# SingleZombie/AFLDM

Measured on AMD Instinct MI355X. Metric: denoise-steps/sec + ms/step, FFHQ-256 AF-UNet, batch 64 @1/2/4/8 GPU, higher is better.
Workload: dtype bf16; 1 GPU; FFHQ-256 AF-UNet single denoise step, batch 64 per GPU (BASELINE configs[1]); batch_per_gpu=64, global_batch=64, hip_graph=True, latents_finite=True

## Files before the change

afldm_amd/_lib.py:

```python
import ctypes
import os
from ctypes import POINTER, Structure, c_char_p, c_float, c_int, c_longlong, c_size_t, c_void_p

import torch

F32, BF16 = 0, 1
DTYPE_CODE = {torch.float32: F32, torch.bfloat16: BF16}

_HERE = os.path.dirname(os.path.abspath(__file__))
LIB_PATH = os.environ.get("AFLDM_LIB") or os.path.join(_HERE, "lib", "libafldm_hip.so")


class ConvArgs(Structure):
    _fields_ = [
        ("x1", c_void_p), ("x2", c_void_p), ("w", c_void_p), ("bias", c_void_p), ("temb", c_void_p),
        ("residual", c_void_p), ("y", c_void_p), ("workspace", c_void_p), ("workspace_bytes", c_size_t),
        ("C1", c_int), ("C2", c_int), ("B", c_int), ("H", c_int), ("W", c_int), ("Cout", c_int),
        ("KS", c_int), ("temb_stride", c_int), ("res_ld", c_int), ("y_ld", c_int),
        ("out_mode", c_int), ("dtype", c_int), ("y2", c_void_p), ("split_n", c_int),
        ("stats_out", c_void_p), ("temb_mod", c_int), ("sync", c_void_p), ("sync_bytes", c_size_t),
        ("defer_reduce", c_int), ("w_batch_stride", ctypes.c_longlong),
        ("y_norm", c_void_p), ("norm_gamma", c_void_p), ("norm_beta", c_void_p), ("norm_groups", c_int), ("norm_eps", c_float),
        ("x_layout", c_int), ("y_layout", c_int),
    ]


class AfActArgs(Structure):
    _fields_ = [
        ("x1", c_void_p), ("x2", c_void_p), ("C1", c_int), ("C2", c_int), ("stats1", c_void_p), ("S1", c_int),
        ("stats2", c_void_p), ("S2", c_int), ("gamma", c_void_p), ("beta", c_void_p), ("G", c_int), ("eps", c_float),
        ("U", c_void_p), ("D", c_void_p), ("packed", c_void_p),
    ]


class SepArgs(Structure):
    _fields_ = [
        ("x", c_void_p), ("y", c_void_p), ("M", c_void_p), ("M2", c_void_p), ("gn_table", c_void_p),
        ("outer_count", ctypes.c_longlong), ("inner_count", ctypes.c_longlong),
# ... 42 lines not shown
        "afldm_af_resample_plane": ([vp, vp, vp, vp, ip, ip, ip, ip, ip, vp], c_int),
        "afldm_upfirdn2d": ([vp, vp, vp] + [ip] * 14 + [fp, ip, vp], c_int),
        "afldm_upfirdn2d_out_size": ([ip] * 6, c_int),
        "afldm_masked_metrics": ([vp, vp, vp, vp, ip, c_size_t, ip, vp], c_int),
        "afldm_gn_fold": ([vp, ip, vp, ip, ip, ip, vp], c_int),
        "afldm_gn_table": ([vp, ip, vp, vp, vp, ip, ip, ip, ip, fp, vp], c_int),
        "afldm_softmax_rows": ([vp, vp, ctypes.c_longlong, ip, fp, ip, vp], c_int),
        "afldm_conv2d": ([POINTER(ConvArgs), vp], c_int),
        "afldm_conv2d_workspace": ([POINTER(ConvArgs)], c_size_t),
        "afldm_conv2d_stats_splits": ([POINTER(ConvArgs)], c_int),
        "afldm_conv2d_tune": ([ip, ip], c_int),
        "afldm_conv2d_fused_splitk": ([ip], c_int),
        "afldm_conv2d_variant": ([POINTER(ConvArgs)], c_int),
        "afldm_conv2d_c8_ok": ([POINTER(ConvArgs)], c_int),
        "afldm_conv2d_norm_ok": ([POINTER(ConvArgs)], c_int),
        "afldm_conv2d_s2": ([POINTER(ConvArgs), ip, ip, vp], c_int),
        "afldm_conv2d_up2": ([POINTER(ConvArgs), vp], c_int),
        "afldm_conv2d_s2_stats_splits": ([POINTER(ConvArgs)], c_int),
        "afldm_conv2d_up2_stats_splits": ([POINTER(ConvArgs)], c_int),
        "afldm_pack_weight_up2": ([vp, vp, ip, ip, ip, vp], c_int),
        "afldm_attention": ([vp, ip, vp, ip, vp, vp, ip, ip, ip, ip, ip, ip, ip, fp, ip, vp], c_int),
        "afldm_attn_block_fused_supported": ([ip, ip, ip, ip], c_int),
        "afldm_attn_block_fused_trace": ([vp], c_int),
        "afldm_af_act_trace": ([vp], c_int),
        "afldm_attn_block_fused": ([vp, vp, ip, vp, vp, ip, fp, vp, vp, vp, ip, ip, ip, ip, fp, ip, vp], c_int),
        "afldm_attn_block_fused_out_supported": ([ip, ip, ip, ip, ip], c_int),
        "afldm_attn_block_fused_out": ([vp, vp, ip, vp, vp, ip, fp, vp, vp, vp, vp, vp, vp, vp, vp, c_longlong, ip, ip, ip, ip, fp, ip,
                                        vp], c_int),
        "afldm_ddim_step": ([vp, vp, vp, vp, vp, ip, ip, ip, ip, ip, ip, vp], c_int),
        "afldm_ddim_step_flat": ([vp, vp, vp, fp, fp, fp, fp, c_size_t, vp], c_int),
# ... 45 lines not shown
```

afldm_amd/csrc/conv.hip:

```cpp
#include <stdlib.h>

#include "conv_common.hpp"

namespace afldm {

__device__ __forceinline__ int swz(int row) { return (4 - ((row >> 2) & 3)) & 3; }

template <typename T>
__device__ __forceinline__ void epilogue_store(const ConvP& p, int m, int n, f32x4 v) {
  const T* temb = (const T*)p.temb;
  const T* res = (const T*)p.residual;
  T* y = (T*)p.y;
  const int HW = p.H * p.W;
  const int b = m / HW;
  if (p.y2 && n >= p.split_n) {
    T* y2 = (T*)p.y2;
    const int pix = m - b * HW, c2 = p.Cout - p.split_n;
    for (int r = 0; r < 4 && n + r < p.Cout; ++r) {
      float sv = v[r] + (p.bias ? p.bias[n + r] : 0.f);
      y2[((size_t)b * c2 + (n + r - p.split_n)) * HW + pix] = from_f32<T>(sv);
    }
    return;
  }
  if (n + 3 < p.Cout && p.vec_ok) {
// ... 1848 lines not shown
    p.stage_ok = ((a->out_mode == 1 || a->y_ld % eo == 0) && (!a->residual || a->res_ld % eo == 0) &&
                  (!a->temb || a->temb_stride % eo == 0) && (!cm || hw % eo == 0) && (!a->y2 || a->split_n % eo == 0) &&
                  !(cm && a->residual)) ? 1 : 0;
    static const int s_nostage = getenv("AFLDM_CONV_NOSTAGE") ? atoi(getenv("AFLDM_CONV_NOSTAGE")) : 0;
    if (s_nostage) p.stage_ok = 0;
  }
  {
    static const int s_mfast = getenv("AFLDM_CONV_MFAST") ? atoi(getenv("AFLDM_CONV_MFAST")) : -1;
    p.m_fast = s_mfast >= 0 ? s_mfast : ((long long)a->Cout * a->KS * a->KS > (long long)p.M ? 1 : 0);
  }
  p.xcd_gn = 0;
  p.y_norm = nullptr; p.ngamma = nullptr; p.nbeta = nullptr; p.ncpg = 1; p.neps = 0.f;
  p.x_c8 = a->x_layout == 1 ? 1 : 0;
  p.y_c8 = a->y_layout == 1 ? 1 : 0;
  p.w_nt = 0;
}

template <typename T>
static bool c8_ok(const afldm_conv_args* a) {
  if (sizeof(T) != 2 || a->C2 != 0 || a->x2 || a->y2 || a->out_mode != 0 || a->y_norm || a->y_ld != a->Cout || a->Cout % 8 || a->C1 % 64) return false;
  if (a->w_batch_stride || a->defer_reduce || a->KS != 3 || lin_wreg_bm(a) || skinny_stats_splits(a)) return false;
  const Exec ex = resolve_exec<T>(a);
  if (ex.pl.kind != 0 || kVariants[ex.vid].ver != 6 || ex.splitk != 1 || ex.fused) return false;
  if (a->stats_out) {
    int S = 0;
    if (stats_mode<T>(a, ex, &S) != ST_EPILOGUE) return false;
  }
  return a->H == a->W && a->W <= 32 && a->H * a->W >= kVariants[ex.vid].bm;
}

template <typename T>
static int conv_dispatch(const afldm_conv_args* a, hipStream_t st) {
  AFLDM_REQUIRE((a->x_layout == 0 && a->y_layout == 0) || c8_ok<T>(a), AFLDM_ESHAPE,
                "afldm_conv2d: x_layout / y_layout = 1 (8-channel blocks) is not available for this problem (afldm_conv2d_c8_ok)");
  ConvP p;
  fill_convp<T>(a, p);
  const Exec ex = resolve_exec<T>(a);
  const Plan& pl = ex.pl;
  int smode = 0;
  p.stats_out = nullptr;
  p.stats_S = 1;
  p.stats_multi = 0;
  if (a->stats_out) smode = stats_mode<T>(a, ex, &p.stats_S);
  int rc = AFLDM_OK;
  AFLDM_REQUIRE(!a->w_batch_stride || pl.kind == 0, AFLDM_ESHAPE, "afldm_conv2d: w_batch_stride needs the GEMM path (Cin a multiple of the K step)");
  if (lin_wreg_bm(a)) return lin_wreg_launch(a, st);
  if (skinny_stats_splits(a)) return skinny_launch(a, st);
  if (pl.kind == 1 && cin4_mfma_ok<T>(a)) {
    if (smode == ST_EPILOGUE) p.stats_out = a->stats_out;
// ... 127 lines not shown
  const long long per = (long long)a->H * a->W * (a->C1 > a->C2 ? a->C1 : a->C2) * esz;
  if (a->B <= 1 || (long long)a->B * per < (1ll << 31) || per >= (1ll << 31)) return a->B;
  int c = (int)(((1ll << 31) - 1) / per);
  while (c > 1 && a->B % c) --c;
  return c;
}

static afldm_conv_args conv_chunk_args(const afldm_conv_args* a, int c) {
  afldm_conv_args q = *a;
  q.B = c;
  return q;
}

template <typename T>
static bool plan_h3(const afldm_conv_args* a, ConvP& p, int& vid) {
  if (conv_batch_chunk(a) != a->B || a->w_batch_stride || a->defer_reduce || a->KS != 3) return false;
  if (lin_wreg_bm(a) || skinny_stats_splits(a)) return false;
  fill_convp<T>(a, p);
  const Exec ex = resolve_exec<T>(a);
  if (ex.pl.kind != 0 || kVariants[ex.vid].ver != 6 || ex.splitk != 1 || ex.fused) return false;
  p.stats_out = nullptr;
  p.stats_S = 1;
  p.stats_multi = 0;
  if (a->stats_out) {
    if (stats_mode<T>(a, ex, &p.stats_S) != ST_EPILOGUE) return false;
    p.stats_out = a->stats_out;
    p.stats_multi = (a->H * a->W) == 1 ? 2 : (a->H * a->W) < kVariants[ex.vid].bm ? 1 : 0;
  }
  p.ksteps = 9 * ((a->C1 + a->C2) / (KCH_DEFAULT * epr<T>()));
  p.splitk = 1;
  p.sync = nullptr;
// ... 21 lines not shown

extern "C" int afldm_conv2d_c8_ok(const afldm_conv_args* a) {
  if (!a || a->dtype != AFLDM_BF16 || conv_validate(a) || conv_batch_chunk(a) != a->B) return 0;
  return c8_ok<bf16>(a) ? 1 : 0;
}

extern "C" int afldm_conv2d_norm_ok(const afldm_conv_args* a) {
  if (!a || a->dtype != AFLDM_BF16 || conv_batch_chunk(a) != a->B || !a->stats_out) return 0;
  if (lin_wreg_bm(a) || skinny_stats_splits(a)) return 0;
  const Exec e = resolve_exec<bf16>(a);
  int S = 0;
  const int smode = stats_mode<bf16>(a, e, &S);
  return norm_fusable<bf16>(a, e, smode) ? 1 : 0;
}

extern "C" int afldm_conv2d_stats_splits(const afldm_conv_args* a0) {
  if (!a0 || (a0->dtype != AFLDM_F32 && a0->dtype != AFLDM_BF16)) return 0;
  const afldm_conv_args ac = conv_chunk_args(a0, conv_batch_chunk(a0));
  const afldm_conv_args* a = &ac;
  int S = 0;
  if (a->dtype == AFLDM_F32) stats_mode<float>(a, resolve_exec<float>(a), &S);
  else stats_mode<bf16>(a, resolve_exec<bf16>(a), &S);
  return S;
}

extern "C" size_t afldm_conv2d_workspace(const afldm_conv_args* a0) {
  if (!a0 || (a0->dtype != AFLDM_F32 && a0->dtype != AFLDM_BF16)) return 0;
  const afldm_conv_args ac = conv_chunk_args(a0, conv_batch_chunk(a0));
  const afldm_conv_args* a = &ac;
  if (lin_wreg_bm(a) || skinny_stats_splits(a)) return 0;
  Plan pl = make_plan(a, a->dtype == AFLDM_F32 ? 16 : 32);
  if (pl.kind != 0 || pl.splitk <= 1) return 0;
  return (size_t)pl.splitk * a->B * a->H * a->W * a->Cout * sizeof(float);
}

extern "C" int afldm_conv2d(const afldm_conv_args* a, afldm_stream_t stream) {
  int rc = conv_validate(a);
  if (rc) return rc;
  hipStream_t st = (hipStream_t)stream;
  if (a->dtype != AFLDM_F32 && a->dtype != AFLDM_BF16) {
    set_error("afldm_conv2d: unknown dtype %d", a->dtype);
    return AFLDM_EDTYPE;
  }
  const int c = conv_batch_chunk(a);
  if (c == a->B) return a->dtype == AFLDM_F32 ? conv_dispatch<float>(a, st) : conv_dispatch<bf16>(a, st);
  const size_t esz = a->dtype == AFLDM_F32 ? 4 : 2;
  const size_t HW = (size_t)a->H * a->W;
  afldm_conv_args q = conv_chunk_args(a, c);
  const int S = a->stats_out ? afldm_conv2d_stats_splits(&q) : 0;
  for (int b0 = 0; b0 < a->B; b0 += c) {
    q.x1 = (const char*)a->x1 + (size_t)b0 * HW * a->C1 * esz;
    q.x2 = a->x2 ? (const char*)a->x2 + (size_t)b0 * HW * a->C2 * esz : nullptr;
    q.y = (char*)a->y + (size_t)b0 * (a->out_mode == 1 ? (size_t)a->Cout * HW : HW * a->y_ld) * esz;
    q.y2 = a->y2 ? (char*)a->y2 + (size_t)b0 * (size_t)(a->Cout - a->split_n) * HW * esz : nullptr;
    q.residual = a->residual ? (const char*)a->residual + (size_t)b0 * HW * a->res_ld * esz : nullptr;
    q.temb = a->temb ? (const char*)a->temb + (size_t)b0 * a->temb_stride * esz : nullptr;
    q.w = (const char*)a->w + (size_t)b0 * (size_t)a->w_batch_stride * esz;
    q.stats_out = a->stats_out ? a->stats_out + (size_t)b0 * S * a->Cout * 2 : nullptr;
    rc = a->dtype == AFLDM_F32 ? conv_dispatch<float>(&q, st) : conv_dispatch<bf16>(&q, st);
// ... 5 lines not shown
```

afldm_amd/csrc/conv3h.hip:

```cpp
#include "conv3h_tile.hpp"

namespace afldm {

template <typename T, int BM, int W_, int BN, int WGM, int WGN, int NPROD, int STAGES, int MINW, int MF, int TPS, bool SUB = false>
__global__ void __launch_bounds__((WGM * WGN + NPROD) * 64, MINW) k_conv3h(ConvP p) {
  extern __shared__ __attribute__((aligned(16))) char smem[];
#define H3_BX blockIdx.x
#define H3_NBX gridDim.x
#define H3_BZ blockIdx.z
#define H3_PATCH_AUX 0
#define H3_PRODUCER_EXIT return;
#include "conv3h_body.inc"
#undef H3_PRODUCER_EXIT
#undef H3_BX
#undef H3_NBX
#undef H3_BZ
#undef H3_PATCH_AUX
}

template <int BM, int W_, int BN, int WGM, int WGN, bool SUB>
__global__ void __launch_bounds__((WGM * WGN + 4) * 64, (WGM * WGN + 4 + 3) / 4) k_conv3h_pers(ConvP p) {
  typedef bf16 T;
  typedef Mma<T> MM;
  typedef typename MM::Chunk Chunk;
// ... 378 lines not shown
  const int kstep = 128 / dtype_size;
  const int eo = 16 / dtype_size;
  const int HW = p.H * p.W;
  const int z = p.splitk > 0 ? p.splitk : 1;
  const bool tile_ok = HW % v.bm == 0 || (v.bm % HW == 0 && (z > 1 || dtype_size == 2));
  const bool plane_ok = v.sub ? (p.W > v.w && p.W % v.w == 0 && p.H % (v.bm / v.w) == 0 && z == 1) : (p.W == v.w && p.H == p.W && tile_ok);
  if ((k == 22 || k == 23) && !(dtype_size == 2 && z == 1 && HW % v.bm == 0 && p.C1 / kstep >= 2 && (!p.temb || p.temb_mod > 0))) return false;
  if (k >= 24 && dtype_size != 2) return false;
  return p.KS == 3 && p.C2 == 0 && plane_ok && p.M % v.bm == 0 && p.Cout % v.bn == 0 &&
         p.C1 % kstep == 0 && (p.C1 / kstep) % z == 0 && p.out_mode == 0 && !p.y2 && p.y_ld % eo == 0 &&
         (!p.residual || p.res_ld % eo == 0) && (!p.temb || (p.temb_stride % eo == 0 && p.temb_mod % eo == 0)) &&
         (long long)p.M * p.C1 * dtype_size < (1ll << 31) && (long long)p.Cout * 9 * p.C1 * dtype_size < (1ll << 31) &&
         p.Cout % 4 == 0 && aligned16(p.y) && aligned16(p.x1) && aligned16(p.w);
}

template <typename T, int BM, int W_, int BN, int WGM, int WGN, int MF, int TPS, int STAGES = 3, bool SUB = false, int NPROD = 4, int MINW_ = 0>
static void launch_h3(const ConvP& p0, hipStream_t st) {
  constexpr int NWC = WGM * WGN;
  constexpr int MINW = MINW_ > 0 ? MINW_ : (NWC + NPROD + 3) / 4;
  constexpr int ROWS = BM / W_, SEG = ROWS < W_ ? ROWS : W_, NSEG = ROWS / SEG;
  constexpr int NPI = (NSEG * (SEG + 2) * (W_ + 2) + 7) / 8;
  constexpr int lds = 2 * NPI * 1024 + STAGES * TPS * BN * 128;
  static_assert(lds <= 160 * 1024, "LDS");
  ConvP p = p0;
  p.tiles_n = p.Cout / BN;
  if (p.splitk < 1) p.splitk = 1;
  const int tiles_m = p.M / BM, tiles = tiles_m * p.tiles_n;
  {
    static const int s_gn = getenv("AFLDM_CONV3H_GN") ? atoi(getenv("AFLDM_CONV3H_GN")) : -1;
    const double xb = (double)p.M * p.C1, wb = 9.0 * p.Cout * p.C1;
// ... 87 lines not shown
```

afldm_amd/csrc/conv3h_body.inc:

```
  typedef Mma<T> MM;
  typedef typename MM::Chunk Chunk;
  constexpr int NWC = WGM * WGN;
  constexpr int EPC = MM::EPC, KSTEP = 8 * EPC, ESZ = (int)sizeof(T);
  constexpr int WMS = BM / WGM, WNS = BN / WGN, TM = WMS / MF, TN = WNS / MF;
  constexpr int ROWS = BM / W_, SEG = ROWS < W_ ? ROWS : W_, NSEG = ROWS / SEG;
  constexpr int PW = W_ + 2, PR = NSEG * (SEG + 2), NPQ = PR * PW, NPI = (NPQ + 7) / 8;
  constexpr int PATCH = NPI * 1024;
  constexpr int SPC = 9 / TPS;
  constexpr int WIT = BN / 8;
  constexpr int WI = TPS * WIT, WPW = WI / NPROD, PPW = (NPI + NPROD - 1) / NPROD;
  constexpr int W_TAP = BN * 128, W_STAGE = TPS * W_TAP;
  constexpr int LDS_TOTAL = 2 * PATCH + STAGES * W_STAGE;
  constexpr unsigned OOB = 0x80000000u;
  static_assert(MF == 16 || MF == 32, "MFMA flavour");
  static_assert(TPS == 1 || TPS == 3, "taps per step");
  static_assert(BM % W_ == 0 && ROWS % SEG == 0 && WI % NPROD == 0 && WMS % MF == 0 && WNS % MF == 0, "tile shape");
  static_assert((STAGES - 2) * WPW + PPW < 64, "vmcnt is a 6-bit counter");

  const int tid = threadIdx.x, lane = tid & 63;
  const int wave_all = __builtin_amdgcn_readfirstlane(tid >> 6);
  const bool is_producer = wave_all >= NWC;
  const int li = lane & (MF - 1), lg = lane / MF;

  int tile_m, tile_n;
// ... 3 lines not shown
    const int xm = xcd / gn, xn = xcd - xm * gn;
    const int lm = j / tn_per, ln = j - lm * tn_per;
    tile_m = xm * tm_per + lm;
    tile_n = xn * tn_per + ln;
  } else {
    const int tile = xcd_remap(H3_BX, H3_NBX);
    tile_m = tile / p.tiles_n;
    tile_n = tile - tile_m * p.tiles_n;
  }
  static_assert(!SUB || (NSEG == 1 && TPS == 1), "sub-tiled planes: one segment per tile");
  const int n0 = tile_n * BN;
  const int Ct = p.C1, HW = SUB ? p.H * p.W : W_ * W_;
  const int ncb = Ct / KSTEP;
  const int ks = H3_BZ;
  const int cb_lo = (ncb * ks) / p.splitk, cb_hi = (ncb * (ks + 1)) / p.splitk;
  const int G = (cb_hi - cb_lo) * SPC;
  int m0, b_tile, oh0, ow0 = 0, sp_tile;
  if constexpr (SUB) {
    const int tw = p.W / W_, tps = (p.H / ROWS) * tw;
    b_tile = tile_m / tps;
    sp_tile = tile_m - b_tile * tps;
    const int ty = sp_tile / tw;
    oh0 = ty * ROWS;
    ow0 = (sp_tile - ty * tw) * W_;
    m0 = b_tile * HW + oh0 * p.W + ow0;
  } else {
    m0 = tile_m * BM;
    b_tile = m0 / HW;
    oh0 = NSEG == 1 ? (m0 - b_tile * HW) / W_ : 0;
    sp_tile = (m0 - b_tile * HW) / BM;
  }
// ... 30 lines not shown
      }
      if (p.x_c8) {
        const int bb = pixel / HW, pp = pixel - bb * HW;
        poff[i] = ok ? (((unsigned)(bb * (Ct / EPC) + c) * (unsigned)HW + (unsigned)pp) * (unsigned)EPC) * ESZ : OOB;
      } else {
        poff[i] = ok ? ((unsigned)pixel * (unsigned)Ct + (unsigned)(c * EPC)) * ESZ : OOB;
      }
    }
#pragma unroll
    for (int i = 0; i < WPW; ++i) {
      const int j = wave + NPROD * i;
      const int tis = j / WIT, r = 8 * (j - tis * WIT) + (lane >> 3);
      const int c = h_chunk_at<MF>(lane & 7, h_sw_rows<MF>(r));
      woff[i] = (((unsigned)(n0 + r) * 9u + (unsigned)tis) * (unsigned)Ct + (unsigned)(c * EPC)) * ESZ;
    }
    int is_g = 0, is_st = 0, is_cb = cb_lo, is_slot = 0;
    auto issue_weights = [&]() {
      char* sbase = smem + 2 * PATCH + is_slot * W_STAGE;
      const unsigned so = is_g < G ? (unsigned)((is_st * TPS * Ct + is_cb * KSTEP) * ESZ) : OOB;
#pragma unroll
      for (int i = 0; i < WPW; ++i) {
        lds_ptr_t dst = (lds_ptr_t)(sbase + (wave + NPROD * i) * 1024);
        if (p.w_nt) __builtin_amdgcn_raw_ptr_buffer_load_lds(rw, dst, 16, (int)woff[i], (int)so, 0, 2);
        else __builtin_amdgcn_raw_ptr_buffer_load_lds(rw, dst, 16, (int)woff[i], (int)so, 0, 0);
      }
      ++is_g;
      if (++is_st == SPC) {
        is_st = 0;
        ++is_cb;
      }
      is_slot = is_slot + 1 == STAGES ? 0 : is_slot + 1;
    };
    auto issue_patch = [&](int cb) {
      char* sbase = smem + ((cb - cb_lo) & 1) * PATCH;
      const unsigned so = p.x_c8 ? (unsigned)cb * (unsigned)(KSTEP * ESZ) * (unsigned)HW : (unsigned)(cb * KSTEP * ESZ);
#pragma unroll
      for (int i = 0; i < PPW; ++i) {
        lds_ptr_t dst = (lds_ptr_t)(sbase + pj[i] * 1024);
        __builtin_amdgcn_raw_ptr_buffer_load_lds(rx, dst, 16, (int)poff[i], (int)so, 0, H3_PATCH_AUX);
      }
    };
    issue_patch(cb_lo);
#pragma unroll
    for (int s = 0; s < STAGES - 1; ++s) issue_weights();
    int st = 0, cb = cb_lo, since = STAGES;
    for (int g = 0; g < G; ++g) {
      if (since <= STAGES - 1) wait_vmcnt<(STAGES - 2) * WPW + PPW>();
      else wait_vmcnt<(STAGES - 2) * WPW>();
      __builtin_amdgcn_s_barrier();
      ++since;
      if (!(p.dbg & 1)) {
        issue_weights();
        if (st == 0 && cb + 1 < cb_hi) {
          issue_patch(cb + 1);
          since = 1;
        }
      }
      if (++st == SPC) {
        st = 0;
        ++cb;
      }
    }
    wait_vmcnt<0>();
    H3_PRODUCER_EXIT
  }

  const int cw = wave_all, wm = cw / WGN, wn = cw - wm * WGN;
  constexpr int NKK = MF == 16 ? 2 : 4;
  constexpr int NACC = MF * MF / 64;
  constexpr int RQ = NACC / 4;
  typedef __attribute__((ext_vector_type(NACC))) float AccT;
  int qb[TM];
#pragma unroll
// ... 191 lines not shown
      }
      static_assert(NRS == 3 || NRS == 8, "peeled steps");
      res_add(NRS - 1);
      g = NRS;
    }
    if constexpr (TPS == 3) {
      for (; g < G; g += 3) {
        __builtin_amdgcn_s_barrier();
        k_step(std::integral_constant<int, 0>{});
        __builtin_amdgcn_s_barrier();
        k_step(std::integral_constant<int, 1>{});
        __builtin_amdgcn_s_barrier();
        k_step(std::integral_constant<int, 2>{});
      }
    } else {
      for (; g < G; ++g) {
        __builtin_amdgcn_s_barrier();
        k_step(RT{});
      }
    }
  }

  if (p.dbg & 8) return;
  if constexpr (ESZ == 2) {
    if (p.splitk == 1) {
      constexpr int NTC = NWC * 64, EO = 8, CPR = BN / EO, RPI = NTC / CPR, OROW = BN + 8;
      constexpr int SB_BYTES = ((NSEG * BN * 4 + 1023) / 1024) * 1024, HWT = BM / NSEG;
      static_assert(SB_BYTES + BM * OROW * 2 <= LDS_TOTAL && RPI * BN * 8 <= LDS_TOTAL, "staging tile");
      float* sB = reinterpret_cast<float*>(smem);
      T* sO = reinterpret_cast<T*>(smem + SB_BYTES);
      const T* temb = (const T*)p.temb;
      const int etid = cw * 64 + lane;
      __syncthreads();
// ... 263 lines not shown
```

afldm_amd/csrc/conv_common.hpp:

```cpp
#pragma once
#include "common.hpp"

namespace afldm {

struct ConvP {
  const void* x1;
  const void* x2;
  const void* w;
  const float* bias;
  const void* temb;
  const void* residual;
  void* y;
  void* y2;
  float* ws;
  int split_n;
  int C1, C2, B, H, W, Cout, KS;
  int temb_stride, res_ld, y_ld, out_mode;
  int temb_mod;
  int M;
  int ksteps;
  int splitk;
  int tiles_n;
  int vec_ok;
  int tap_inner;
// ... 1 lines not shown
  int stats_S;
  int stats_multi;
  int m_fast;
  int stage_ok;
  int dbg;
  int xcd_gn;
  unsigned* sync;
  long long w_bstride;
  void* y_norm;
  const float* ngamma;
  const float* nbeta;
  int ncpg;
  float neps;
  int x_c8, y_c8;
  int w_nt;
};

typedef __attribute__((address_space(3))) void* lds_ptr_t;

template <int N>
__device__ __forceinline__ void wait_vmcnt() {
  asm volatile("s_waitcnt vmcnt(%0)" ::"n"(N) : "memory");
}

constexpr int kConv3hFirst = 41;
bool conv3h_supported(int variant, int dtype_size, const ConvP& p);
int conv3h_tile(int variant, int* bm, int* bn);
void conv3h_launch(int variant, int dtype_size, const ConvP& p, hipStream_t st);
bool conv3h_plan(const afldm_conv_args* a, ConvP* p, int* variant);

}
```

afldm_amd/models/blocks.py:

```python
import math

import os

import torch
import torch.nn as nn

from .. import aql, ops

_SC_ORDER = int(os.environ.get("AFLDM_SHORTCUT_ORDER", "0"))
_C8_EDGES = int(os.environ.get("AFLDM_C8_EDGES", "5"))


def _pair(x):
    return x if isinstance(x, tuple) else (x, None)


class PackedMixin:

    def _packed(self, key, build):
        cache = self.__dict__.setdefault("_afldm_cache", {})
        if key not in cache:
            cache[key] = build()
        return cache[key]

    def _invalidate(self):
# ... 325 lines not shown
                or tuple(self.conv1.kernel_size) != (3, 3) or tuple(self.conv2.kernel_size) != (3, 3)):
            return False, False
        B, N = x1.shape[0], x1.shape[1]
        cin = x1.shape[-1] + (0 if x2 is None else x2.shape[-1])
        key = (B, N, cin, x1.device, int(temb_stride))
        cache = self.__dict__.setdefault("_afldm_c8", {})
        if key not in cache:
            w1, b1 = packed_conv(self.conv1, x1.dtype)
            w2, b2 = packed_conv(self.conv2, x1.dtype)
            a_in = torch.empty((B, N, N, cin), dtype=x1.dtype, device=x1.device)
            h_in = torch.empty((B, N, N, self.out_channels), dtype=x1.dtype, device=x1.device)
            cache[key] = (ops.conv2d_c8_ok(a_in, w1, b1, temb=temb_proj, temb_stride=temb_stride),
                          ops.conv2d_c8_ok(h_in, w2, b2, residual=h_in))
        return cache[key]

    def _norm_act(self, norm, x, out_c8=False, out_const=False):
        from ..af_modules.af_blocks import WarpedNonlinearity
        x1, x2 = _pair(x)
        gamma, beta = packed_norm(norm)
        stats = ops.gn_stats(x1, norm.num_groups, x2=x2)
        if isinstance(self.nonlinearity, WarpedNonlinearity):
            if self.nonlinearity.fused_silu:
                return ops.af_act(x1, x2, stats, gamma, beta, norm.num_groups, norm.eps, out_c8=out_c8, out_const=out_const)
            return self.nonlinearity(ops.gn_apply(x1, stats, gamma, beta, norm.num_groups, norm.eps, act=0, x2=x2))
        return ops.gn_apply(x1, stats, gamma, beta, norm.num_groups, norm.eps, act=1, x2=x2)

    def _norm_act_conv(self, norm, x, conv, force=False, **kw):
        from ..af_modules.af_blocks import WarpedNonlinearity
        x1, x2 = _pair(x)
        if (isinstance(self.nonlinearity, WarpedNonlinearity) and self.nonlinearity.fused_silu and x1.ndim == 4
# ... 112 lines not shown
        return _plane2_view(y, B, Cout)

    def forward(self, input_tensor, temb_proj=None, temb_stride=0, next_gn=None):
        x1, x2 = _pair(input_tensor)
        if self._const2_ok(input_tensor):
            return self._forward_const2(input_tensor, temb_proj, temb_stride, next_gn)
        if x1.ndim == 4 and x1.shape[1] in ops._ACTCONV_N:
            h = self._norm_act_conv(self.norm1, input_tensor, self.conv1, temb=temb_proj, temb_stride=temb_stride, want_stats=True)
            res = conv_forward(self.conv_shortcut, input_tensor) if self.conv_shortcut is not None else x1
            assert self.conv_shortcut is not None or x2 is None
            return self._norm_act_conv(self.norm2, h, self.conv2, residual=res, want_stats=True)
        c8_1, c8_2 = self._c8_plan(input_tensor, temb_proj, temb_stride)
        e1, e2, e3 = c8_1 and bool(_C8_EDGES & 1), c8_1 and bool(_C8_EDGES & 2), c8_2 and bool(_C8_EDGES & 4)
        res = None
        merged1 = bool(ops._ACTCONV_SITES) and x1.ndim == 4 and (x1.shape[1], x1.shape[-1] + (0 if x2 is None else x2.shape[-1])) in ops._ACTCONV_SITES
        if merged1:
            h = None
        elif self.conv_shortcut is not None and _SC_ORDER == 2:
            res = conv_forward(self.conv_shortcut, input_tensor)
            with aql.independent("act1"):
                h = self._norm_act(self.norm1, input_tensor, out_c8=e1)
        else:
            h = self._norm_act(self.norm1, input_tensor, out_c8=e1)
        if self.conv_shortcut is not None and _SC_ORDER == 1:
            with aql.independent("shortcut"):
                res = conv_forward(self.conv_shortcut, input_tensor)
        fused = self._conv1_norm2_act_fused(h, temb_proj, temb_stride) if h is not None else None
        if fused is not None:
            h = fused
        elif h is None:
            h = self._norm_act_conv(self.norm1, input_tensor, self.conv1, force=True, temb=temb_proj, temb_stride=temb_stride, want_stats=True)
            h = self._norm_act(self.norm2, h, out_c8=e3)
        else:
            h = conv_forward(self.conv1, h, temb=temb_proj, temb_stride=temb_stride, want_stats=True, out_c8=e2)
            h = self._norm_act(self.norm2, h, out_c8=e3)
        if res is not None:
            pass
        elif self.conv_shortcut is not None:
            with aql.independent("shortcut"):
                res = conv_forward(self.conv_shortcut, input_tensor)
        else:
            assert x2 is None
            res = x1
        if next_gn is not None:
            out = self._conv2_to_next_norm_fused(h, res, next_gn)
            if out is not None:
                return out
            gamma, beta = packed_norm(next_gn)
            out = conv_forward(self.conv2, h, residual=res, want_stats=True,
                               norm_out=(gamma, beta, next_gn.num_groups, next_gn.eps))
# ... 210 lines not shown
```

afldm_amd/ops.py:

```python
import ctypes
import os

import torch

from . import _exp, _lib
from ._lib import AfActArgs, ConvArgs, DTYPE_CODE, SepArgs, check, stream_ptr

_FILTER_CACHE = {}
_PROFILE = None


class _RecordingLib:

    def __init__(self, raw):
        self._raw = raw
        self._wrapped = {}

    def __getattr__(self, name):
        w = self._wrapped.get(name)
        if w is None:
            f = getattr(self._raw, name)

            def w(*a, _f=f):
                if _PROFILE is not None:
# ... 651 lines not shown
        return False
    key = (tuple(x1.shape), tuple(w.shape), temb is not None, int(temb_stride), residual is not None, bool(want_stats), str(x1.device))
    if key not in _C8_OK:
        a = conv_args(x1, w, bias, None, temb, temb_stride, residual, None)
        a.y = ptr(x1)
        if want_stats and w.shape[0] % 4 == 0:
            a.stats_out = ptr(x1)
        a.x_layout = 0
        _C8_OK[key] = (not lib.afldm_conv2d_workspace(ctypes.byref(a))) and bool(lib.afldm_conv2d_c8_ok(ctypes.byref(a)))
    return _C8_OK[key]


_C8_OK = {}


def conv2d(x1, w, bias=None, x2=None, temb=None, temb_stride=0, residual=None, out=None, out_mode=0,
           workspace=None, want_stats=False, temb_mod=0, w_batch_stride=0, norm_out=None, out_c8=False):
    Cout = w.shape[0]
    if out is None:
        if out_mode == 0:
            out = torch.empty(tuple(x1.shape[:-1]) + (Cout,), dtype=x1.dtype, device=x1.device)
        else:
            B = x1.shape[0]
            out = torch.empty((B, Cout, x1.numel() // (B * x1.shape[-1])), dtype=x1.dtype, device=x1.device)
    a = conv_args(x1, w, bias, x2, temb, temb_stride, residual, out, out_mode, workspace, temb_mod=temb_mod)
    if out_c8:
        a.y_layout = 1
        out.c8 = True
    a.w_batch_stride = int(w_batch_stride)
    if out_mode == 1 and x1.ndim == 3:
        a.B, a.H, a.W = x1.shape[0], x1.shape[1], 1
    if workspace is None:
        need = lib.afldm_conv2d_workspace(ctypes.byref(a))
        if need:
            workspace = torch.empty(need // 4, dtype=torch.float32, device=x1.device)
            a.workspace, a.workspace_bytes = ptr(workspace), need
    st = None
    if want_stats and out_mode == 0 and Cout % 4 == 0:
        S = lib.afldm_conv2d_stats_splits(ctypes.byref(a))
        st = torch.empty((a.B, S, Cout, 2), dtype=torch.float32, device=x1.device)
        a.stats_out = ptr(st)
    hn = None
    if norm_out is not None and _CONV_NORM and st is not None:
        gamma, beta, G, eps = norm_out
# ... 4 lines not shown
            a.keep = a.keep + (hn, gamma, beta)
    tok = _begin()
    check(lib.afldm_conv2d(ctypes.byref(a), stream_ptr()), "conv2d")
    if hn is not None:
        out.norm_applied = hn
    if st is not None:
        if st.shape[1] > _MAX_SPLITS and st.shape[1] % _MAX_SPLITS == 0:
            folded = torch.empty((a.B, _MAX_SPLITS, Cout, 2), dtype=torch.float32, device=x1.device)
            check(lib.afldm_gn_fold(ptr(st), st.shape[1], ptr(folded), _MAX_SPLITS, a.B, Cout, stream_ptr()), "gn_fold")
            st = folded
        out.gn_partial = st
    if tok is not None:
        M, Ct = a.B * a.H * a.W, a.C1 + a.C2
        es = x1.element_size()
        kind = "conv3x3" if a.KS == 3 else ("conv1x1" if a.H * a.W > 1 and x1.ndim == 4 else "linear")
        keep = (a, st, out, workspace)
        _end(tok, kind, 2.0 * M * a.Cout * a.KS * a.KS * Ct,
             (M * Ct + a.Cout * a.KS * a.KS * Ct + M * a.Cout * (2 if residual is not None else 1)) * es,
             replay=lambda keep=keep: conv2d_launch(keep[0]))
    return out


_ACTCONV = os.environ.get("AFLDM_NO_ACTCONV", "0") != "1"
_ACTCONV_N = tuple(int(v) for v in os.environ.get("AFLDM_ACTCONV_N", "").split(",") if v)
_ACTCONV_SITES = frozenset(tuple(int(x) for x in v.split(":")) for v in os.environ.get("AFLDM_ACTCONV_SITES", "").split(",") if v)


def act_conv_act(x1, x2, pre, w, bias=None, temb=None, temb_stride=0, residual=None, want_stats=False, post=None):
    if (not _ACTCONV or not _exp.available() or x1.ndim != 4 or x1.dtype != torch.bfloat16 or x1.shape[1] != x1.shape[2] or x1.shape[1] not in (16, 32)
            or (pre is None and post is None)):
        return None
    C1, x2, C2 = _cat_args(x1, x2)
    B, N = x1.shape[0], x1.shape[1]
# ... 485 lines not shown
```

include/afldm_hip.h:

```cpp
#ifndef AFLDM_HIP_H
#define AFLDM_HIP_H

#include <stddef.h>
#include <stdint.h>

#ifdef __cplusplus
extern "C" {
#endif

typedef void* afldm_stream_t;

enum { AFLDM_F32 = 0, AFLDM_BF16 = 1 };
enum {
  AFLDM_OK = 0,
  AFLDM_ESHAPE = -1,
  AFLDM_EDTYPE = -2,
  AFLDM_EALIGN = -3,
  AFLDM_ELAUNCH = -4,
  AFLDM_ENULL = -5
};

int afldm_version(void);
const char* afldm_last_error(void);
int afldm_device_info(char* name, int name_len);
// ... 101 lines not shown
  void* y2;
  int split_n;
  float* stats_out;
  int temb_mod;
  unsigned int* sync;
  size_t sync_bytes;
  int defer_reduce;
  long long w_batch_stride;
  void* y_norm;
  const float* norm_gamma;
  const float* norm_beta;
  int norm_groups;
  float norm_eps;
  int x_layout;
  int y_layout;
} afldm_conv_args;
int afldm_conv2d(const afldm_conv_args* args, afldm_stream_t stream);
int afldm_conv2d_c8_ok(const afldm_conv_args* args);
int afldm_conv2d_norm_ok(const afldm_conv_args* args);
int afldm_conv2d_tune(int variant, int splitk);
int afldm_conv2d_fused_splitk(int enable);
int afldm_conv2d_variant(const afldm_conv_args* args);
size_t afldm_conv2d_workspace(const afldm_conv_args* args);
int afldm_conv2d_stats_splits(const afldm_conv_args* args);

int afldm_conv2d_s2(const afldm_conv_args* args, int pad_lo, int pad_hi, afldm_stream_t stream);
int afldm_conv2d_up2(const afldm_conv_args* args, afldm_stream_t stream);
int afldm_conv2d_s2_stats_splits(const afldm_conv_args* args);
int afldm_conv2d_up2_stats_splits(const afldm_conv_args* args);
int afldm_pack_weight_up2(const float* src, void* dst, int Cout, int Cin, int dtype, afldm_stream_t stream);

int afldm_attention(const void* q, int ldq, const void* k, int ldk, const void* vt, void* o, int ldo,
                    int B, int Bk, int heads, int Tq, int Tk, int d, float scale, int dtype,
                    afldm_stream_t stream);
// ... 49 lines not shown
```

Before: 13100 denoise-steps/s.

## Fold 1x1 shortcut conv into the resnet conv2 3x3 implicit GEMM K-loop

Extends the conv3h kernel so that extra K-steps after the 3x3 reduction load the block input and the packed 1x1 shortcut weights. The shortcut projection is then accumulated into the same output tile, with the two biases summed on the host side. This removes a separate shortcut conv launch and the write and re-read of its output as a residual tensor. In exchange it adds pipeline-wait logic for the new K-steps and only applies to eligible single-split variants. It is on by default where the plan check succeeds.

```diff
diff --git a/afldm_amd/_lib.py b/afldm_amd/_lib.py
--- a/afldm_amd/_lib.py
+++ b/afldm_amd/_lib.py
@@ -22,6 +22,7 @@
         ("defer_reduce", c_int), ("w_batch_stride", ctypes.c_longlong),
         ("y_norm", c_void_p), ("norm_gamma", c_void_p), ("norm_beta", c_void_p), ("norm_groups", c_int), ("norm_eps", c_float),
         ("x_layout", c_int), ("y_layout", c_int),
+        ("sc_x1", c_void_p), ("sc_x2", c_void_p), ("sc_w", c_void_p), ("sc_C1", c_int), ("sc_C2", c_int),
     ]
 
 
@@ -94,6 +95,7 @@
         "afldm_conv2d_variant": ([POINTER(ConvArgs)], c_int),
         "afldm_conv2d_c8_ok": ([POINTER(ConvArgs)], c_int),
         "afldm_conv2d_norm_ok": ([POINTER(ConvArgs)], c_int),
+        "afldm_conv2d_shortcut_ok": ([POINTER(ConvArgs)], c_int),
         "afldm_conv2d_s2": ([POINTER(ConvArgs), ip, ip, vp], c_int),
         "afldm_conv2d_up2": ([POINTER(ConvArgs), vp], c_int),
         "afldm_conv2d_s2_stats_splits": ([POINTER(ConvArgs)], c_int),
diff --git a/afldm_amd/csrc/conv.hip b/afldm_amd/csrc/conv.hip
--- a/afldm_amd/csrc/conv.hip
+++ b/afldm_amd/csrc/conv.hip
@@ -1886,6 +1886,23 @@
   p.x_c8 = a->x_layout == 1 ? 1 : 0;
   p.y_c8 = a->y_layout == 1 ? 1 : 0;
   p.w_nt = 0;
+  p.sc_x1 = a->sc_x1; p.sc_x2 = a->sc_x2; p.sc_w = a->sc_w;
+  p.sc_C1 = a->sc_x1 ? a->sc_C1 : 0; p.sc_C2 = a->sc_x1 ? a->sc_C2 : 0;
+}
+
+template <typename T>
+static bool shortcut_ok(const afldm_conv_args* a) {
+  const int kstep = KCH_DEFAULT * epr<T>();
+  const long long M = (long long)a->B * a->H * a->W, Csc = (long long)a->sc_C1 + a->sc_C2;
+  if (!a->sc_x1 || !a->sc_w || a->sc_C1 <= 0 || a->sc_C2 < 0 || a->sc_C1 % kstep || a->sc_C2 % kstep || (a->sc_C2 > 0) != (a->sc_x2 != nullptr))
+    return false;
+  if (!aligned16(a->sc_x1) || !aligned16(a->sc_x2) || !aligned16(a->sc_w)) return false;
+  if (a->KS != 3 || a->residual || a->defer_reduce || a->w_batch_stride || a->y_norm || a->y2 || a->out_mode != 0) return false;
+  const long long cmax = a->sc_C1 > a->sc_C2 ? a->sc_C1 : a->sc_C2;
+  if (M >= (1ll << 28) || M * cmax * (long long)sizeof(T) >= (1ll << 31) || (long long)a->Cout * Csc * (long long)sizeof(T) >= (1ll << 31)) return false;
+  if (lin_wreg_bm(a) || skinny_stats_splits(a)) return false;
+  const Exec ex = resolve_exec<T>(a);
+  return ex.pl.kind == 0 && kVariants[ex.vid].ver == 6 && ex.splitk == 1 && !ex.fused && conv3h_shortcut_ok(ex.vid);
 }
 
 template <typename T>
@@ -1905,6 +1922,8 @@
 static int conv_dispatch(const afldm_conv_args* a, hipStream_t st) {
   AFLDM_REQUIRE((a->x_layout == 0 && a->y_layout == 0) || c8_ok<T>(a), AFLDM_ESHAPE,
                 "afldm_conv2d: x_layout / y_layout = 1 (8-channel blocks) is not available for this problem (afldm_conv2d_c8_ok)");
+  AFLDM_REQUIRE(!a->sc_x1 || shortcut_ok<T>(a), AFLDM_ESHAPE,
+                "afldm_conv2d: the folded shortcut (sc_x1 / sc_w) is not available for this problem (afldm_conv2d_shortcut_ok)");
   ConvP p;
   fill_convp<T>(a, p);
   const Exec ex = resolve_exec<T>(a);
@@ -2062,7 +2081,7 @@
 
 template <typename T>
 static bool plan_h3(const afldm_conv_args* a, ConvP& p, int& vid) {
-  if (conv_batch_chunk(a) != a->B || a->w_batch_stride || a->defer_reduce || a->KS != 3) return false;
+  if (conv_batch_chunk(a) != a->B || a->w_batch_stride || a->defer_reduce || a->KS != 3 || a->sc_x1) return false;
   if (lin_wreg_bm(a) || skinny_stats_splits(a)) return false;
   fill_convp<T>(a, p);
   const Exec ex = resolve_exec<T>(a);
@@ -2114,6 +2133,13 @@
   return norm_fusable<bf16>(a, e, smode) ? 1 : 0;
 }
 
+extern "C" int afldm_conv2d_shortcut_ok(const afldm_conv_args* a) {
+  if (!a || conv_validate(a) || conv_batch_chunk(a) != a->B) return 0;
+  if (a->dtype == AFLDM_BF16) return shortcut_ok<bf16>(a) ? 1 : 0;
+  if (a->dtype == AFLDM_F32) return shortcut_ok<float>(a) ? 1 : 0;
+  return 0;
+}
+
 extern "C" int afldm_conv2d_stats_splits(const afldm_conv_args* a0) {
   if (!a0 || (a0->dtype != AFLDM_F32 && a0->dtype != AFLDM_BF16)) return 0;
   const afldm_conv_args ac = conv_chunk_args(a0, conv_batch_chunk(a0));
@@ -2143,6 +2169,7 @@
     return AFLDM_EDTYPE;
   }
   const int c = conv_batch_chunk(a);
+  AFLDM_REQUIRE(!a->sc_x1 || c == a->B, AFLDM_ESHAPE, "afldm_conv2d: the folded shortcut needs the whole batch in one launch");
   if (c == a->B) return a->dtype == AFLDM_F32 ? conv_dispatch<float>(a, st) : conv_dispatch<bf16>(a, st);
   const size_t esz = a->dtype == AFLDM_F32 ? 4 : 2;
   const size_t HW = (size_t)a->H * a->W;
diff --git a/afldm_amd/csrc/conv3h.hip b/afldm_amd/csrc/conv3h.hip
--- a/afldm_amd/csrc/conv3h.hip
+++ b/afldm_amd/csrc/conv3h.hip
@@ -416,6 +416,13 @@
          p.Cout % 4 == 0 && aligned16(p.y) && aligned16(p.x1) && aligned16(p.w);
 }
 
+bool conv3h_shortcut_ok(int variant) {
+  const int k = variant - kConv3hFirst;
+  if (k < 0 || k >= kNumH3 || k == 22 || k == 23) return false;
+  const H3Variant& v = kH3[k];
+  return v.bm != 0 && v.tps == 1 && !v.sub && !(v.bm == 256 && v.w == 16);
+}
+
 template <typename T, int BM, int W_, int BN, int WGM, int WGN, int MF, int TPS, int STAGES = 3, bool SUB = false, int NPROD = 4, int MINW_ = 0>
 static void launch_h3(const ConvP& p0, hipStream_t st) {
   constexpr int NWC = WGM * WGN;
diff --git a/afldm_amd/csrc/conv3h_body.inc b/afldm_amd/csrc/conv3h_body.inc
--- a/afldm_amd/csrc/conv3h_body.inc
+++ b/afldm_amd/csrc/conv3h_body.inc
@@ -41,7 +41,10 @@
   const int ncb = Ct / KSTEP;
   const int ks = H3_BZ;
   const int cb_lo = (ncb * ks) / p.splitk, cb_hi = (ncb * (ks + 1)) / p.splitk;
-  const int G = (cb_hi - cb_lo) * SPC;
+  constexpr bool HAS_SC = TPS == 1 && !SUB && !(BM == 256 && W_ == 16);
+  const int nsc = (HAS_SC && p.sc_x1) ? (p.sc_C1 + p.sc_C2) / KSTEP : 0;
+  const int cb_end = cb_hi + nsc;
+  const int Gm = (cb_hi - cb_lo) * SPC, G = Gm + nsc;
   int m0, b_tile, oh0, ow0 = 0, sp_tile;
   if constexpr (SUB) {
     const int tw = p.W / W_, tps = (p.H / ROWS) * tw;
@@ -102,15 +105,29 @@
       const int c = h_chunk_at<MF>(lane & 7, h_sw_rows<MF>(r));
       woff[i] = (((unsigned)(n0 + r) * 9u + (unsigned)tis) * (unsigned)Ct + (unsigned)(c * EPC)) * ESZ;
     }
+    const int Csc = p.sc_C1 + p.sc_C2;
+    __amdgpu_buffer_rsrc_t rws = __builtin_amdgcn_make_buffer_rsrc((void*)p.sc_w, 0, (int)((long long)p.Cout * Csc * ESZ), 0x00020000);
     int is_g = 0, is_st = 0, is_cb = cb_lo, is_slot = 0;
     auto issue_weights = [&]() {
       char* sbase = smem + 2 * PATCH + is_slot * W_STAGE;
-      const unsigned so = is_g < G ? (unsigned)((is_st * TPS * Ct + is_cb * KSTEP) * ESZ) : OOB;
-#pragma unroll
-      for (int i = 0; i < WPW; ++i) {
-        lds_ptr_t dst = (lds_ptr_t)(sbase + (wave + NPROD * i) * 1024);
-        if (p.w_nt) __builtin_amdgcn_raw_ptr_buffer_load_lds(rw, dst, 16, (int)woff[i], (int)so, 0, 2);
-        else __builtin_amdgcn_raw_ptr_buffer_load_lds(rw, dst, 16, (int)woff[i], (int)so, 0, 0);
+      if (HAS_SC && is_g >= Gm && is_g < G) {
+        const unsigned so = (unsigned)((is_g - Gm) * KSTEP * ESZ);
+#pragma unroll
+        for (int i = 0; i < WPW; ++i) {
+          const int r = 8 * (wave + NPROD * i) + (lane >> 3);
+          const unsigned wo = ((unsigned)(n0 + r) * (unsigned)Csc + (unsigned)(h_chunk_at<MF>(lane & 7, h_sw_rows<MF>(r)) * EPC)) * ESZ;
+          lds_ptr_t dst = (lds_ptr_t)(sbase + (wave + NPROD * i) * 1024);
+          if (p.w_nt) __builtin_amdgcn_raw_ptr_buffer_load_lds(rws, dst, 16, (int)wo, (int)so, 0, 2);
+          else __builtin_amdgcn_raw_ptr_buffer_load_lds(rws, dst, 16, (int)wo, (int)so, 0, 0);
+        }
+      } else {
+        const unsigned so = is_g < Gm ? (unsigned)((is_st * TPS * Ct + is_cb * KSTEP) * ESZ) : OOB;
+#pragma unroll
+        for (int i = 0; i < WPW; ++i) {
+          lds_ptr_t dst = (lds_ptr_t)(sbase + (wave + NPROD * i) * 1024);
+          if (p.w_nt) __builtin_amdgcn_raw_ptr_buffer_load_lds(rw, dst, 16, (int)woff[i], (int)so, 0, 2);
+          else __builtin_amdgcn_raw_ptr_buffer_load_lds(rw, dst, 16, (int)woff[i], (int)so, 0, 0);
+        }
       }
       ++is_g;
       if (++is_st == SPC) {
@@ -121,6 +138,27 @@
     };
     auto issue_patch = [&](int cb) {
       char* sbase = smem + ((cb - cb_lo) & 1) * PATCH;
+      if (HAS_SC && cb >= cb_hi) {
+        const int c0 = (cb - cb_hi) * KSTEP;
+        const bool in1 = c0 < p.sc_C1;
+        const int Cs = in1 ? p.sc_C1 : p.sc_C2;
+        __amdgpu_buffer_rsrc_t rs = __builtin_amdgcn_make_buffer_rsrc(const_cast<void*>(in1 ? p.sc_x1 : p.sc_x2), 0,
+                                                                     (int)((long long)p.M * Cs * ESZ), 0x00020000);
+        const unsigned so = (unsigned)((in1 ? c0 : c0 - p.sc_C1) * ESZ);
+#pragma unroll
+        for (int i = 0; i < PPW; ++i) {
+          const int q = 8 * pj[i] + (lane >> 3);
+          const int c = h_chunk_at<MF>(lane & 7, h_sw_patch<MF, W_>(q));
+          const int pr = q / PW, pc = q - pr * PW;
+          const int sg = pr / (SEG + 2), jj = pr - sg * (SEG + 2);
+          const bool in = q < NPQ && pc >= 1 && pc <= W_ && jj >= 1 && jj <= SEG;
+          const int pixel = m0 + (sg * SEG + jj - 1) * W_ + (pc - 1);
+          const unsigned off = in ? ((unsigned)pixel * (unsigned)Cs + (unsigned)(c * EPC)) * ESZ : OOB;
+          lds_ptr_t dst = (lds_ptr_t)(sbase + pj[i] * 1024);
+          __builtin_amdgcn_raw_ptr_buffer_load_lds(rs, dst, 16, (int)off, (int)so, 0, 0);
+        }
+        return;
+      }
       const unsigned so = p.x_c8 ? (unsigned)cb * (unsigned)(KSTEP * ESZ) * (unsigned)HW : (unsigned)(cb * KSTEP * ESZ);
 #pragma unroll
       for (int i = 0; i < PPW; ++i) {
@@ -132,19 +170,31 @@
 #pragma unroll
     for (int s = 0; s < STAGES - 1; ++s) issue_weights();
     int st = 0, cb = cb_lo, since = STAGES;
+    bool fresh = false;
     for (int g = 0; g < G; ++g) {
-      if (since <= STAGES - 1) wait_vmcnt<(STAGES - 2) * WPW + PPW>();
+      if (fresh) wait_vmcnt<(STAGES >= 3 ? WPW : 0)>();
+      else if (since <= STAGES - 1) wait_vmcnt<(STAGES - 2) * WPW + PPW>();
       else wait_vmcnt<(STAGES - 2) * WPW>();
       __builtin_amdgcn_s_barrier();
       ++since;
+      fresh = false;
       if (!(p.dbg & 1)) {
-        issue_weights();
-        if (st == 0 && cb + 1 < cb_hi) {
-          issue_patch(cb + 1);
-          since = 1;
-        }
-      }
-      if (++st == SPC) {
+        if (HAS_SC && cb >= cb_hi) {
+          if (cb + 1 < cb_end) {
+            issue_patch(cb + 1);
+            fresh = true;
+            since = STAGES;
+          }
+          issue_weights();
+        } else {
+          issue_weights();
+          if (st == 0 && cb + 1 < cb_end) {
+            issue_patch(cb + 1);
+            since = 1;
+          }
+        }
+      }
+      if ((HAS_SC && cb >= cb_hi) || ++st == SPC) {
         st = 0;
         ++cb;
       }
@@ -366,9 +416,16 @@
         k_step(std::integral_constant<int, 2>{});
       }
     } else {
-      for (; g < G; ++g) {
+      for (; g < Gm; ++g) {
         __builtin_amdgcn_s_barrier();
         k_step(RT{});
+      }
+      for (; HAS_SC && g < G; ++g) {
+        __builtin_amdgcn_s_barrier();
+        st = 4;
+        k_step(RT{});
+        st = 0;
+        pbuf ^= 1;
       }
     }
   }
diff --git a/afldm_amd/csrc/conv_common.hpp b/afldm_amd/csrc/conv_common.hpp
--- a/afldm_amd/csrc/conv_common.hpp
+++ b/afldm_amd/csrc/conv_common.hpp
@@ -39,6 +39,10 @@
   float neps;
   int x_c8, y_c8;
   int w_nt;
+  const void* sc_x1;
+  const void* sc_x2;
+  const void* sc_w;
+  int sc_C1, sc_C2;
 };
 
 typedef __attribute__((address_space(3))) void* lds_ptr_t;
@@ -50,6 +54,7 @@
 
 constexpr int kConv3hFirst = 41;
 bool conv3h_supported(int variant, int dtype_size, const ConvP& p);
+bool conv3h_shortcut_ok(int variant);
 int conv3h_tile(int variant, int* bm, int* bn);
 void conv3h_launch(int variant, int dtype_size, const ConvP& p, hipStream_t st);
 bool conv3h_plan(const afldm_conv_args* a, ConvP* p, int* variant);
diff --git a/afldm_amd/models/blocks.py b/afldm_amd/models/blocks.py
--- a/afldm_amd/models/blocks.py
+++ b/afldm_amd/models/blocks.py
@@ -9,6 +9,7 @@
 
 _SC_ORDER = int(os.environ.get("AFLDM_SHORTCUT_ORDER", "0"))
 _C8_EDGES = int(os.environ.get("AFLDM_C8_EDGES", "5"))
+_SC_FOLD = os.environ.get("AFLDM_NO_SHORTCUT_FOLD", "0") != "1"
 
 
 def _pair(x):
@@ -364,6 +365,49 @@
                           ops.conv2d_c8_ok(h_in, w2, b2, residual=h_in))
         return cache[key]
 
+    def _sc_bias(self):
+        cache = self.__dict__.setdefault("_afldm_cache", {})
+        if "sc_bias" not in cache:
+            b = torch.zeros(self.out_channels, dtype=torch.float64, device=self.conv2.weight.device)
+            for conv in (self.conv2, self.conv_shortcut):
+                if conv.bias is not None:
+                    b += conv.bias.detach().double()
+            cache["sc_bias"] = b.float().contiguous()
+        return cache["sc_bias"]
+
+    def _sc_fold_plan(self, input_tensor, c8):
+        if (not _SC_FOLD or self.conv_shortcut is None or tuple(self.conv_shortcut.kernel_size) != (1, 1)
+                or tuple(self.conv2.kernel_size) != (3, 3)):
+            return False
+        x1, x2 = _pair(input_tensor)
+        if x1.ndim != 4 or x1.shape[1] != x1.shape[2]:
+            return False
+        B, N = x1.shape[0], x1.shape[1]
+        key = (B, N, x1.shape[-1], None if x2 is None else x2.shape[-1], x1.dtype, x1.device, bool(c8))
+        cache = self.__dict__.setdefault("_afldm_sc_fold", {})
+        if key not in cache:
+            w2, _ = packed_conv(self.conv2, x1.dtype)
+            wsc, _ = packed_conv(self.conv_shortcut, x1.dtype)
+            h_in = torch.empty((B, N, N, self.out_channels), dtype=x1.dtype, device=x1.device)
+            if c8:
+                h_in.c8 = True
+            cache[key] = ops.conv2d_shortcut_ok(h_in, w2, self._sc_bias(), (x1, x2, wsc))
+        return cache[key]
+
+    def _conv2_sc_folded(self, h, input_tensor, next_gn):
+        x1, x2 = _pair(input_tensor)
+        w2, _ = packed_conv(self.conv2, h.dtype)
+        wsc, _ = packed_conv(self.conv_shortcut, h.dtype)
+        kw = {}
+        if next_gn is not None:
+            gamma, beta = packed_norm(next_gn)
+            kw["norm_out"] = (gamma, beta, next_gn.num_groups, next_gn.eps)
+        out = ops.conv2d(h, w2, self._sc_bias(), want_stats=True, shortcut=(x1, x2, wsc), **kw)
+        hn = getattr(out, "norm_applied", None)
+        if hn is not None:
+            out.gn_applied = (hn, next_gn)
+        return out
+
     def _norm_act(self, norm, x, out_c8=False, out_const=False):
         from ..af_modules.af_blocks import WarpedNonlinearity
         x1, x2 = _pair(x)
@@ -506,15 +550,16 @@
         e1, e2, e3 = c8_1 and bool(_C8_EDGES & 1), c8_1 and bool(_C8_EDGES & 2), c8_2 and bool(_C8_EDGES & 4)
         res = None
         merged1 = bool(ops._ACTCONV_SITES) and x1.ndim == 4 and (x1.shape[1], x1.shape[-1] + (0 if x2 is None else x2.shape[-1])) in ops._ACTCONV_SITES
+        fold = not merged1 and self._sc_fold_plan(input_tensor, e3)
         if merged1:
             h = None
-        elif self.conv_shortcut is not None and _SC_ORDER == 2:
+        elif self.conv_shortcut is not None and _SC_ORDER == 2 and not fold:
             res = conv_forward(self.conv_shortcut, input_tensor)
             with aql.independent("act1"):
                 h = self._norm_act(self.norm1, input_tensor, out_c8=e1)
         else:
             h = self._norm_act(self.norm1, input_tensor, out_c8=e1)
-        if self.conv_shortcut is not None and _SC_ORDER == 1:
+        if self.conv_shortcut is not None and _SC_ORDER == 1 and not fold:
             with aql.independent("shortcut"):
                 res = conv_forward(self.conv_shortcut, input_tensor)
         fused = self._conv1_norm2_act_fused(h, temb_proj, temb_stride) if h is not None else None
@@ -526,6 +571,8 @@
         else:
             h = conv_forward(self.conv1, h, temb=temb_proj, temb_stride=temb_stride, want_stats=True, out_c8=e2)
             h = self._norm_act(self.norm2, h, out_c8=e3)
+        if fold:
+            return self._conv2_sc_folded(h, input_tensor, next_gn)
         if res is not None:
             pass
         elif self.conv_shortcut is not None:
diff --git a/afldm_amd/ops.py b/afldm_amd/ops.py
--- a/afldm_amd/ops.py
+++ b/afldm_amd/ops.py
@@ -689,8 +689,36 @@
 _C8_OK = {}
 
 
+def _set_shortcut(a, shortcut):
+    sx1, sx2, sw = shortcut
+    _dev(sx1, "shortcut x1")
+    assert not is_c8(sx1) and not is_c8(sx2), "the folded shortcut reads NHWC tensors"
+    a.sc_x1, a.sc_x2, a.sc_w = ptr(sx1), ptr(sx2), ptr(sw)
+    a.sc_C1, a.sc_C2 = sx1.shape[-1], 0 if sx2 is None else sx2.shape[-1]
+    a.keep = a.keep + (sx1, sx2, sw)
+
+
+def conv2d_shortcut_ok(x1, w, bias, shortcut, temb=None, temb_stride=0, want_stats=True):
+    sx1, sx2, sw = shortcut
+    if x1.ndim != 4 or sx1.ndim != 4 or w.shape[1] != 3 or sw.shape[1] != 1:
+        return False
+    key = (tuple(x1.shape), is_c8(x1), x1.dtype, tuple(w.shape), tuple(sx1.shape), None if sx2 is None else tuple(sx2.shape),
+           temb is not None, int(temb_stride), bool(want_stats), str(x1.device))
+    if key not in _SC_OK:
+        a = conv_args(x1, w, bias, None, temb, temb_stride, None, None)
+        a.y = ptr(sx1)
+        if want_stats and w.shape[0] % 4 == 0:
+            a.stats_out = ptr(sx1)
+        _set_shortcut(a, shortcut)
+        _SC_OK[key] = (not lib.afldm_conv2d_workspace(ctypes.byref(a))) and bool(lib.afldm_conv2d_shortcut_ok(ctypes.byref(a)))
+    return _SC_OK[key]
+
+
+_SC_OK = {}
+
+
 def conv2d(x1, w, bias=None, x2=None, temb=None, temb_stride=0, residual=None, out=None, out_mode=0,
-           workspace=None, want_stats=False, temb_mod=0, w_batch_stride=0, norm_out=None, out_c8=False):
+           workspace=None, want_stats=False, temb_mod=0, w_batch_stride=0, norm_out=None, out_c8=False, shortcut=None):
     Cout = w.shape[0]
     if out is None:
         if out_mode == 0:
@@ -703,6 +731,8 @@
         a.y_layout = 1
         out.c8 = True
     a.w_batch_stride = int(w_batch_stride)
+    if shortcut is not None:
+        _set_shortcut(a, shortcut)
     if out_mode == 1 and x1.ndim == 3:
         a.B, a.H, a.W = x1.shape[0], x1.shape[1], 1
     if workspace is None:
@@ -737,9 +767,10 @@
         M, Ct = a.B * a.H * a.W, a.C1 + a.C2
         es = x1.element_size()
         kind = "conv3x3" if a.KS == 3 else ("conv1x1" if a.H * a.W > 1 and x1.ndim == 4 else "linear")
+        Csc = a.sc_C1 + a.sc_C2 if shortcut is not None else 0
         keep = (a, st, out, workspace)
-        _end(tok, kind, 2.0 * M * a.Cout * a.KS * a.KS * Ct,
-             (M * Ct + a.Cout * a.KS * a.KS * Ct + M * a.Cout * (2 if residual is not None else 1)) * es,
+        _end(tok, kind, 2.0 * M * a.Cout * (a.KS * a.KS * Ct + Csc),
+             (M * (Ct + Csc) + a.Cout * (a.KS * a.KS * Ct + Csc) + M * a.Cout * (2 if residual is not None else 1)) * es,
              replay=lambda keep=keep: conv2d_launch(keep[0]))
     return out
 
diff --git a/include/afldm_hip.h b/include/afldm_hip.h
--- a/include/afldm_hip.h
+++ b/include/afldm_hip.h
@@ -139,10 +139,15 @@
   float norm_eps;
   int x_layout;
   int y_layout;
+  const void* sc_x1;
+  const void* sc_x2;
+  const void* sc_w;
+  int sc_C1, sc_C2;
 } afldm_conv_args;
 int afldm_conv2d(const afldm_conv_args* args, afldm_stream_t stream);
 int afldm_conv2d_c8_ok(const afldm_conv_args* args);
 int afldm_conv2d_norm_ok(const afldm_conv_args* args);
+int afldm_conv2d_shortcut_ok(const afldm_conv_args* args);
 int afldm_conv2d_tune(int variant, int splitk);
 int afldm_conv2d_fused_splitk(int enable);
 int afldm_conv2d_variant(const afldm_conv_args* args);
```

Measured after the change: 13480 denoise-steps/s, median of 6. 2.9% higher.
